# intel/QATzip

Hardware: AMD Instinct MI355X
Metric: compress + decompress GB/s (input bytes), QZ_DEFLATE_GZIP_EXT L1, 64 KB chunks (higher is better)
Workload: dtype u8

## Files before the change

### qatzip_amd/csrc/qzd_inflate.hip

```cpp
#include <algorithm>
#include <atomic>
#include <chrono>
#include <condition_variable>
#include <functional>
#include <mutex>
#include <thread>
#include <string.h>
#include <string>
#include <vector>

#include "qzd_internal.h"
#include <stdlib.h>
#include "qzk_inflate.h"
#include "qzk_inflate_lane.h"
#include "qzk_inflate_spec.h"
#include "qzk_checksum.h"
#include "qzd_inflate_plan.h"
#include <stddef.h>

static_assert(sizeof(qzp_seg) == sizeof(qzk_infseg) && offsetof(qzp_seg, in_off) == offsetof(qzk_infseg, in_off) &&
              offsetof(qzp_seg, out_off) == offsetof(qzk_infseg, out_off) && offsetof(qzp_seg, in_len) == offsetof(qzk_infseg, in_len) &&
              offsetof(qzp_seg, out_cap) == offsetof(qzk_infseg, out_cap) && offsetof(qzp_seg, flags) == offsetof(qzk_infseg, flags) &&
              offsetof(qzp_seg, pad) == offsetof(qzk_infseg, pad), "qzp_seg mirrors qzk_infseg");
static_assert(sizeof(qzp_res) == sizeof(qzk_infres) && offsetof(qzp_res, status) == offsetof(qzk_infres, status) &&
              offsetof(qzp_res, in_used) == offsetof(qzk_infres, in_used) && offsetof(qzp_res, out_len) == offsetof(qzk_infres, out_len) &&
              offsetof(qzp_res, nblocks) == offsetof(qzk_infres, nblocks), "qzp_res mirrors qzk_infres");
static_assert(QZP_FINAL == QZK_INF_FINAL && QZP_FLUSH == QZK_INF_FLUSH && QZP_TOKSEG_BYTES == sizeof(qzk_tokseg), "qzd_inflate_plan.h's constants");

#define QZD_LANE_MIN_SEGS 1024u
#define QZD_LANE_MIN_SEGS_BIG 2048u
#define QZD_LANE_MIN(seg_bytes) ((seg_bytes) <= 65536u + 64u ? QZD_LANE_MIN_SEGS : QZD_LANE_MIN_SEGS_BIG)
#define QZD_LANE_SEGS_PER_WAVE 16u
#define QZD_SPEC_LANES 4u
#define QZD_SPEC_LANES_FEW 8u
#define QZD_SPEC_FEW_SEGS 16384u
#define QZD_SPEC_FEW_SEGS_BIG 32768u
#define QZD_SPEC_LANES_FEWER 16u
#define QZD_SPEC_FEWER_SEGS 8192u
static uint32_t spec_lanes(const qzk_infseg *hs, uint32_t nsegs)
{
    const bool big = hs[0].out_cap > 16384u + 64u, upto512 = hs[0].out_cap <= 524288u + 64u;
    uint32_t K = nsegs <= QZD_SPEC_FEWER_SEGS && hs[0].out_cap > 131072u + 64u && upto512 ? 32u
// ... 98 lines not shown
struct tp_host { qzk_infseg *segs; qzk_infres *res; qzk_tokseg *ts; uint32_t *ord; };
static tp_host tp_host_of(qzd_ctx *c, const tp_mirror &M)
{
    return tp_host{(qzk_infseg *)c->h_aux, (qzk_infres *)(c->h_aux + M.o_res), (qzk_tokseg *)(c->h_aux + M.o_ts), (uint32_t *)(c->h_aux + M.o_ord)};
}
struct tp_dev {
    qzk_infseg *segs; qzk_infres *res; qzk_inf_tab *tab; qzk_tokseg *ts; qzk_chain *ch; qzk_rec *rec;
    uint8_t *lit; qzk_seq *seq; uint32_t *ord;
};

struct tp_plan {
    bool uniform; qzk_tsfill F;
    uint64_t arena;
    uint64_t hb0, hb_rg; uint32_t R;
};
static int plan_regions(qzd_ctx *c, const qzk_infseg *hs, uint32_t nsegs, uint32_t K, qzk_tokseg *tsv, tp_plan *pl)
{
    uint64_t arena = 0, max_cap = 0;
    qzk_tsfill &F = pl->F;
    bool uniform = nsegs > 0 && K <= 32;
    for (uint32_t i = 0; i < nsegs && uniform; i++) uniform = !(hs[i].flags & QZK_INF_COUNT_ONLY) && hs[i].out_cap == hs[0].out_cap;
    if (uniform) {
        F.seg = 0; max_cap = hs[0].out_cap;
        for (uint32_t j = 0; j < K; j++) {
            F.len[j] = K == 1 ? QZK_TOK_REGION(hs[0].out_cap) : QZK_SPEC_REGION(hs[0].out_cap, K, j);
            F.pre[j] = F.seg; F.seg += F.len[j];
        }
        arena = (uint64_t)nsegs * F.seg;
    } else
    for (uint32_t i = 0; i < nsegs; i++) {
        const bool writes = !(hs[i].flags & QZK_INF_COUNT_ONLY);
        if (writes && hs[i].out_cap > max_cap) max_cap = hs[i].out_cap;
        for (uint32_t j = 0; j < K; j++) {
            const uint64_t rg = !writes ? 0 : K == 1 ? QZK_TOK_REGION(hs[i].out_cap) : QZK_SPEC_REGION(hs[i].out_cap, K, j);
            tsv[(size_t)i * K + j].lit_off = arena; tsv[(size_t)i * K + j].seq_off = (arena + rg) / 8;
            arena += rg;
        }
    }
    pl->uniform = uniform;
    pl->R = K == 1 ? 0u : std::min<uint32_t>(nsegs, QZK_SPEC_HANDBACK(nsegs));
    pl->hb0 = arena; pl->hb_rg = QZK_TOK_REGION(max_cap);
    pl->arena = arena + (uint64_t)pl->R * pl->hb_rg;
    bool aligned = ((pl->hb0 | pl->hb_rg) & 15) == 0;
    if (uniform) for (uint32_t j = 0; j < K; j++) aligned &= ((F.pre[j] | F.len[j] | F.seg) & 15) == 0;
    else for (size_t i = 0; i < (size_t)nsegs * K; i++) aligned &= ((tsv[i].lit_off & 15) | (tsv[i].seq_off & 1)) == 0;
    if (!aligned) { snprintf(c->err, sizeof(c->err), "inflate: a token region is not 16-byte aligned"); return QZD_ERR_PARAM; }
    return QZD_OK;
}
static void fill_host(const tp_plan &pl, qzk_tokseg *tsv, uint32_t nsegs, uint32_t K)
{
    for (uint32_t i = 0; i < nsegs; i++)
        for (uint32_t j = 0; j < K; j++) {
            const uint64_t a = (uint64_t)i * pl.F.seg + pl.F.pre[j];
            tsv[(size_t)i * K + j].lit_off = a; tsv[(size_t)i * K + j].seq_off = (a + pl.F.len[j]) / 8;
        }
// ... 9 lines not shown
    c->d_big = NULL; c->big_cap = 0;
    const char *cap_e = getenv("QATZIP_AMD_SCRATCH_MAX");
    const bool refused = cap_e && need > (size_t)strtoull(cap_e, NULL, 10);
    if (refused || hipMalloc(&c->d_big, need) != hipSuccess) {
        (void)hipGetLastError();
        c->d_big = NULL;
        return QZD_ERR_NOMEM;
    }
    c->big_cap = need;
    return QZD_OK;
}

#ifndef QZD_TOK_OCC
#define QZD_TOK_OCC 2
#endif
static void tok_launch(hipStream_t st, const uint8_t *d_comp, const tp_dev &D, uint32_t nsegs, uint32_t K, const uint32_t *order, uint32_t count)
{
    uint32_t lpw = QZD_LANE_SEGS_PER_WAVE;
    const char *le = getenv("QATZIP_AMD_INFLATE_LPW");
    if (le) { int v = atoi(le); if (v == 8 || v == 16 || v == 32 || v == 64) lpw = (uint32_t)v; }
    const char *oe = getenv("QATZIP_AMD_INFLATE_OCC");
    const int occ = oe ? atoi(oe) : 0;
    const dim3 grid(((order ? count : nsegs) + lpw - 1) / lpw), blk(lpw);
#define QZD_TOK_LAUNCH(N, W) hipLaunchKernelGGL((qzk_inflate_tok_kernel<N, W>), grid, blk, 0, st, d_comp, D.segs, D.res, nsegs, D.tab, \
                                               D.ts, D.lit, D.seq, D.ch, order, count, K)
    switch (lpw) {
    case 8: if (occ == 2) QZD_TOK_LAUNCH(8, 2); else QZD_TOK_LAUNCH(8, 4); break;
    case 32: QZD_TOK_LAUNCH(32, 1); break;
    case 64: QZD_TOK_LAUNCH(64, 1); break;
    default: QZD_TOK_LAUNCH(16, QZD_TOK_OCC);
    }
#undef QZD_TOK_LAUNCH
}
static void spec_launch(qzd_ctx *c, hipStream_t st, const uint8_t *d_comp, const tp_dev &D, const qzk_infseg *hs, uint32_t nsegs, uint32_t K)
{
    const uint32_t spw = 64 / K;
    const dim3 grid((nsegs + spw - 1) / spw), blk(64);
    static std::atomic<uint64_t> spec_epoch{0};
    const uint64_t epoch = ++spec_epoch;
    uint32_t over = hs[0].out_cap > 65536u + 64u ? 2u : nsegs <= 4096u ? 1u : 1000u;
// ... 67 lines not shown
        c->so_sent = off[parts];
    }
    return QZD_OK;
}

static int fetch_results(qzd_ctx *c, qzk_infres *st_res, const qzk_infres *d_res, uint32_t nsegs, qzk_infres *h_res, hipStream_t st)
{
    const size_t rb = (size_t)nsegs * sizeof(qzk_infres);
    HIPCHK(c, ctl_copy(st_res, d_res, rb, st));
    HIPCHK(c, hipStreamSynchronize(st));
    HIPCHK(c, hipGetLastError());
    memcpy(h_res, st_res, rb);
    return QZD_OK;
}

static int two_phase(qzd_ctx *c, const uint8_t *d_comp, uint8_t *d_out, const qzk_infseg *hs, uint32_t nsegs,
                     qzk_infres *h_res, uint32_t K, hipStream_t st, bool run_b = true)
{
    const tp_mirror M = tp_mirror_of(nsegs, K);
    int rc = qzd_aux_reserve(c, M.bytes + 64);
    if (rc) return rc;
    const tp_host H = tp_host_of(c, M);
    const size_t sb = (size_t)nsegs * sizeof(qzk_infseg);
    memcpy(H.segs, hs, sb);
    tp_plan pl;
    rc = plan_regions(c, hs, nsegs, K, H.ts, &pl);
    if (rc) return rc;
    const size_t tabb = ((size_t)nsegs * sizeof(qzk_inf_tab) + 255) & ~(size_t)255;
    const size_t tsb = ((size_t)nsegs * K * sizeof(qzk_tokseg) + 255) & ~(size_t)255;
    const size_t chb = ((size_t)nsegs * sizeof(qzk_chain) + 255) & ~(size_t)255;
    const size_t rcb = K == 1 ? 0 : (((size_t)nsegs * K * QZK_SPEC_NREC * sizeof(qzk_rec) + 255) & ~(size_t)255);
    const size_t litb = (pl.arena + 1023) & ~(uint64_t)255;
    const size_t ordb = ((size_t)nsegs * 4 + 255) & ~(size_t)255;
    const size_t need = tabb + tsb + chb + rcb + litb + ordb + 256;
    const bool stream_out = run_b && c->so_host && c->so_nat && nsegs >= QZD_LANE_MIN_SEGS;
    if (big_reserve(c, need, st) != QZD_OK) {
        if (K > 1) return two_phase(c, d_comp, d_out, hs, nsegs, h_res, 1, st, run_b);
        snprintf(c->err, sizeof(c->err), "inflate: %zu bytes of decode scratch are not available", need);
        return QZD_ERR_NOMEM;
    }
    tp_dev D;
    uint8_t *pb = c->d_big;
    D.segs = (qzk_infseg *)c->d_aux; D.res = (qzk_infres *)(c->d_aux + M.o_res);
    D.tab = (qzk_inf_tab *)pb; pb += tabb;
    D.ts = (qzk_tokseg *)pb; pb += tsb;
    D.ch = (qzk_chain *)pb; pb += chb;
    D.rec = (qzk_rec *)pb; pb += rcb;
    D.lit = pb; pb += litb;
    D.seq = (qzk_seq *)D.lit;
    D.ord = (uint32_t *)pb;
    HIPCHK(c, ctl_copy(D.segs, H.segs, sb, st));
    if (pl.uniform) {
        hipLaunchKernelGGL(qzk_ts_fill_kernel, dim3((unsigned)std::min<size_t>(((size_t)nsegs * K + 255) / 256, 1024)), dim3(256), 0, st, D.ts, nsegs, K, pl.F);
        HIPCHK(c, hipGetLastError());
    } else HIPCHK(c, ctl_copy(D.ts, H.ts, (size_t)nsegs * K * sizeof(qzk_tokseg), st));
    HIPCHK(c, hipEventRecord(c->ev[1][1], st));
    bool res_fresh = false;
    if (K == 1) tok_launch(st, d_comp, D, nsegs, K, NULL, 0);
    else {
        spec_launch(c, st, d_comp, D, hs, nsegs, K);
        uint32_t nredo = 0;
        rc = handback_redo(c, st, d_comp, pl, H, D, nsegs, K, &nredo);
        if (rc) return rc;
        if (nredo > pl.R) {
            c->inf_k1rerun_acc++;
            return two_phase(c, d_comp, d_out, hs, nsegs, h_res, 1, st, run_b);
        }
        res_fresh = nredo == 0;
    }
    HIPCHK(c, hipEventRecord(c->ev[1][0], st));
// ... 260 lines not shown
}

static void build_candidates(const std::vector<uint32_t> &start, uint64_t n, uint32_t avail, uint32_t shift, uint32_t seg_hint,
                             std::vector<qzk_infseg> &ps, std::vector<uint32_t> &where)
{
    const uint32_t ns = (uint32_t)ps.size();
    std::vector<uint32_t> order(ns);
    order_by_clen(start, n, shift, order);
    for (uint32_t i = 0; i < ns; i++) {
        const uint32_t k = order[i];
        where[k] = i;
        ps[i].in_off = start[k]; ps[i].in_len = avail - start[k];
        ps[i].out_off = 0; ps[i].out_cap = seg_hint; ps[i].flags = 0; ps[i].pad = clen(start.data(), (uint32_t)start.size(), n, k);
    }
}
static void seat_links(const qzp_walk &W, const std::vector<uint32_t> &where, std::vector<qzk_infseg> &ps, std::vector<uint32_t> &chain)
{
    for (qzk_infseg &s : ps) s.flags = QZK_INF_COUNT_ONLY;
    for (const qzp_link &l : W.links) {
        qzk_infseg &s = ps[where[l.cand]];
        s.out_off = l.out_off; s.out_cap = l.out_len; s.flags = 0;
        chain.push_back(where[l.cand]);
    }
}

#define QZD_PATH_DONE 1
#define QZD_PATH_NEXT 2
#define QZD_PATH_LANES_NOMEM 3
struct inf_lap {
    bool on; std::chrono::steady_clock::time_point prev;
    void operator()(const char *what)
    {
        if (!on) return;
        auto t = std::chrono::steady_clock::now();
        fprintf(stderr, "[qzd_inflate_stream] %-22s %8.3f ms\n", what, std::chrono::duration<double, std::milli>(t - prev).count());
        prev = t;
    }
};
struct inf_call {
    qzd_ctx *c; const uint8_t *d_src; uint64_t n; uint8_t *d_dst; uint64_t dst_cap; uint32_t seg_hint;
    uint8_t *h_dst; int *h_sent;
    bool scan_ok; std::vector<uint32_t> start; uint32_t ns;
    bool lanes, lanes_nomem;
    std::vector<qzk_infseg> segs; std::vector<qzk_infres> res;
    uint64_t total_out, total_in;
    inf_lap lap;
};

static int path_lanes(inf_call &S)
{
    qzd_ctx *c = S.c;
    const uint32_t ns = S.ns;
    static const bool lone_lanes = getenv("QATZIP_AMD_LONE_WAVE") == NULL;
    if (!(S.scan_ok && S.seg_hint && (ns > 1 || (lone_lanes && S.seg_hint > 16384u)) && S.lanes)) return QZD_PATH_NEXT;
    static const uint32_t cls_shift = cls_shift_of(getenv("QATZIP_AMD_INFLATE_CLS"));
    std::vector<qzk_infseg> ps(ns);
    std::vector<qzk_infres> pr(ns);
    std::vector<uint32_t> where(ns);
    build_candidates(S.start, S.n, (uint32_t)S.n, cls_shift, S.seg_hint, ps, where);
    S.lap("segment records");
    HIPCHK(c, hipEventRecord(c->ev[0][0], c->st[0]));
    int rc = two_phase(c, S.d_src, S.d_dst, ps.data(), ns, pr.data(), spec_lanes(ps.data(), ns), c->st[0], false);
    if (rc == QZD_ERR_NOMEM) return QZD_PATH_LANES_NOMEM;
    if (rc) return rc;
    S.lap("phase A");
    const qzp_walk W = chain_walk(S.start.data(), ns, ns, (const qzp_res *)pr.data(), where.data(), 0, 0, S.dst_cap);
    if (!W.ok) return QZD_PATH_NEXT;
    if (W.over < W.links.size()) return QZD_ERR_DSTCAP;
    std::vector<uint32_t> chain;
    seat_links(W, where, ps, chain);
    c->so_sent = 0;
    rc = two_phase_resolve(c, S.d_src, S.d_dst, ps.data(), ns, chain.data(), (uint32_t)chain.size(), pr.data(), S.h_dst, c->st[0]);
    if (rc) return rc;
    bool ok = true;
    for (uint32_t i : chain) if (pr[i].status < 0) { ok = false; break; }
    HIPCHK(c, hipEventRecord(c->ev[0][1], c->st[0]));
    HIPCHK(c, hipStreamSynchronize(c->st[0]));
    float t = 0;
    if (hipEventElapsedTime(&t, c->ev[0][0], c->ev[0][1]) == hipSuccess) c->inf_ms[0] += t;
    S.lap("phase B");
// ... 83 lines not shown
}

static int inflate_stream(qzd_ctx *c, const uint8_t *d_src, uint64_t n, uint8_t *d_dst, uint64_t dst_cap,
                          uint32_t seg_hint, uint64_t *h_in_used, uint64_t *h_out_len, uint32_t *h_crc, uint8_t *h_dst, int *h_sent)
{
    if (h_sent) *h_sent = 0;
    if (!c || !d_src || !h_in_used || !h_out_len) return QZD_ERR_PARAM;
    if (n == 0 || n > 0xffffffffull) return QZD_ERR_PARAM;
    hipSetDevice(c->device);
    c->inf_ms[0] = c->inf_ms[1] = c->inf_ms[2] = c->inf_ms[3] = 0;
    *h_in_used = 0; *h_out_len = 0;
    static const bool trace = getenv("QATZIP_AMD_TRACE") != NULL;
    inf_call S;
    S.c = c; S.d_src = d_src; S.n = n; S.d_dst = d_dst; S.dst_cap = dst_cap; S.seg_hint = seg_hint; S.h_dst = h_dst; S.h_sent = h_sent;
    S.total_out = S.total_in = 0;
    S.lap.on = trace; S.lap.prev = std::chrono::steady_clock::now();
    std::vector<uint32_t> mk;
    int rc = find_markers(c, d_src, n, mk);
    S.lap("marker scan + sort");
    if (rc < 0) return rc;
    S.scan_ok = rc == 0;
    S.start.push_back(0);
    if (S.scan_ok) for (uint32_t p : mk) if (p < n) S.start.push_back(p);
    S.ns = (uint32_t)S.start.size();
    const char *force_path = getenv("QATZIP_AMD_INFLATE");
    S.lanes = force_path ? force_path[0] == 'l' : true;
    S.lanes_nomem = false;
    rc = path_lanes(S);
    if (rc == QZD_PATH_LANES_NOMEM) { S.lanes_nomem = true; rc = QZD_PATH_NEXT; }
    if (rc == QZD_PATH_NEXT) { S.segs.resize(S.ns); S.res.resize(S.ns); rc = path_optimistic(S); }
    if (rc == QZD_PATH_NEXT) rc = path_two_pass(S);
    if (rc == QZD_PATH_NEXT) rc = path_one_wave(S);
    if (rc != QZD_PATH_DONE) return rc;
    *h_in_used = S.total_in; *h_out_len = S.total_out;
    S.lap("chain check / rest");
    if (h_crc) { rc = qzd_crc32(c, d_dst, S.total_out, h_crc); S.lap("crc32"); return rc; }
    return QZD_OK;
}

extern "C" int qzd_inflate_stream(qzd_ctx *c, const uint8_t *d_src, uint64_t n, uint8_t *d_dst, uint64_t dst_cap,
                                  uint32_t seg_hint, uint64_t *h_in_used, uint64_t *h_out_len, uint32_t *h_crc)
{
    return inflate_stream(c, d_src, n, d_dst, dst_cap, seg_hint, h_in_used, h_out_len, h_crc, NULL, NULL);
}

extern "C" int qzd_inflate_stream_to_host(qzd_ctx *c, const uint8_t *d_src, uint64_t n, uint8_t *d_dst, uint64_t dst_cap,
                                          uint32_t seg_hint, uint64_t *h_in_used, uint64_t *h_out_len, uint32_t *h_crc,
                                          uint8_t *h_dst, int *h_sent)
{
    if (!h_dst || !h_sent) return QZD_ERR_PARAM;
// ... 256 lines not shown
```

### qatzip_amd/csrc/qzd_inflate_plan.h

```cpp
#ifndef QZD_INFLATE_PLAN_H
#define QZD_INFLATE_PLAN_H
#include <stdint.h>
#include <stdlib.h>
#include <algorithm>
#include <vector>

struct qzp_seg { uint64_t in_off, out_off; uint32_t in_len, out_cap, flags, pad; };
struct qzp_res { int32_t status; uint32_t in_used, out_len, nblocks; };
#define QZP_FINAL 0
#define QZP_FLUSH 1
#define QZP_TOKSEG_BYTES 16u

static inline uint32_t clen(const uint32_t *start, uint32_t ns, uint64_t n, uint32_t k)
{
    return (k + 1 < ns ? start[k + 1] : (uint32_t)n) - start[k];
}

#define QZP_CLASSES 8192u
static inline void order_by_clen(const std::vector<uint32_t> &start, uint64_t n, uint32_t shift, std::vector<uint32_t> &order)
{
    const uint32_t ns = (uint32_t)order.size(), nstart = (uint32_t)start.size();
    std::vector<uint32_t> cnt(QZP_CLASSES + 1, 0);
    auto rcls = [&](uint32_t k) { const uint32_t v = clen(start.data(), nstart, n, k) >> shift; return QZP_CLASSES - 1 - (v < QZP_CLASSES ? v : QZP_CLASSES - 1); };
    for (uint32_t i = 0; i < ns; i++) cnt[rcls(i) + 1]++;
    for (uint32_t i = 0; i < QZP_CLASSES; i++) cnt[i + 1] += cnt[i];
    for (uint32_t i = 0; i < ns; i++) order[cnt[rcls(i)]++] = i;
// ... 27 lines not shown
        W.links.push_back(qzp_link{k, oo, r.out_len});
        oo += r.out_len;
        if (oo > cap && W.over == (size_t)-1) W.over = W.links.size() - 1;
        if (r.status == QZP_FINAL) { W.final = true; W.total_in = (uint64_t)start[k] + r.in_used; break; }
        W.next = start[k] + r.in_used;
        uint32_t j = k + 1;
        while (j < nstart && start[j] < W.next) j++;
        if (j >= nstart || start[j] != W.next) { W.ok = false; break; }
        k = j;
    }
    W.oo = oo;
    if (W.over == (size_t)-1) W.over = W.links.size();
    return W;
}

#define QZD_PIPE_MAX 8u
#define QZD_PIPE_FIRST_PCT 3u
#define QZD_PIPE_MIN_BYTES (12u << 20)
#define QZD_PIPE_GROW_NUM 9u
#define QZD_PIPE_GROW_DEN 5u
static inline void pipe_plan(uint64_t n, uint64_t cut[QZD_PIPE_MAX + 1], uint32_t *P_out)
{
    uint64_t len = std::max<uint64_t>(n * QZD_PIPE_FIRST_PCT / 100, QZD_PIPE_MIN_BYTES), at = 0;
    uint32_t P = 0;
    cut[0] = 0;
    while (P + 1 < QZD_PIPE_MAX && at + len + len / 2 < n) {
        at = (at + len) & ~(uint64_t)4095; cut[++P] = at;
        len = len * QZD_PIPE_GROW_NUM / QZD_PIPE_GROW_DEN;
    }
    cut[++P] = n;
// ... 36 lines not shown
```

### qatzip_amd/csrc/qzk_checksum.h

```cpp
#ifndef QZK_CHECKSUM_H
#define QZK_CHECKSUM_H
#include "qzk_deflate_huff.h"

typedef struct { uint64_t off; uint32_t len; uint32_t pad; } qzk_range;

QZ_KERNEL qzk_crc_kernel(const uint8_t *data, const qzk_range *ranges, uint32_t nranges, uint32_t *crc_out)
{
    QZ_LDS qzk_crc_lds S;
    const uint32_t r = blockIdx.x;
    if (r >= nranges) return;
    const uint32_t c = qzk_block_crc32(&S, data + ranges[r].off, ranges[r].len);
    if (threadIdx.x == 0) crc_out[r] = c;
}

QZ_KERNEL qzk_crc_chunks_kernel(const uint8_t *src, uint64_t src_len, uint32_t chunk_sz, uint32_t nchunks, uint32_t *crc_out,
                                const uint32_t *cdesc )
{
    QZ_LDS qzk_crc_lds S;
    const uint32_t c = blockIdx.x;
    if (c >= nchunks) return;
    const uint64_t off = (uint64_t)c * chunk_sz;
    const uint32_t n = cdesc ? (cdesc[c] & 0x7fffffffu) : (uint32_t)((src_len - off) < chunk_sz ? (src_len - off) : chunk_sz);
    const uint32_t v = qzk_block_crc32(&S, src + off, n);
    if (threadIdx.x == 0) crc_out[c] = v;
}

#define QZK_ADLER_MOD 65521u
QZ_KERNEL qzk_adler_chunks_kernel(const uint8_t *src, uint64_t src_len, uint32_t chunk_sz, uint32_t nchunks, uint32_t *out)
{
    QZ_LDS uint32_t pa[QZK_HT], pb[QZK_HT];
    const uint32_t c = blockIdx.x, t = threadIdx.x;
    if (c >= nchunks) return;
    const uint64_t off = (uint64_t)c * chunk_sz;
    const uint32_t n = (uint32_t)((src_len - off) < chunk_sz ? (src_len - off) : chunk_sz);
    const uint32_t S = (n + QZK_HT - 1) / QZK_HT;
    const uint32_t b0 = t * S < n ? t * S : n, b1 = (t + 1) * S < n ? (t + 1) * S : n;
// ... 18 lines not shown
```

### qatzip_amd/csrc/qzk_inflate_lane.h

```cpp
#ifndef QZK_INFLATE_LANE_H
#define QZK_INFLATE_LANE_H
#include "qzk_inflate.h"
#include "qzk_lz_batch.h"

#ifdef QZ_SIM
#define QZK_PIN(x) ((void)0)
#else
#define QZK_PIN(x) asm volatile("" : "+v"(x))
#endif

#ifndef QZK_LLROOT
#define QZK_LLROOT 9
#endif
#ifndef QZK_LDROOT
#define QZK_LDROOT 7
#endif
#define QZK_CLROOT 7
#define QZK_SIDE_BYTES 256
#define QZK_SIDE_SPARE 28
#define QZK_LPOOL_N (QZK_SIDE_BYTES - (1 << QZK_LDROOT) - QZK_SIDE_SPARE)
#define QZK_LANE_ROOTSZ ((1 << QZK_LLROOT) + QZK_SIDE_BYTES / 2)
#define QZK_DROOT8(droot) ((uint8_t *)(droot))
#define QZK_LPOOL(droot) ((uint8_t *)(droot) + (1 << QZK_LDROOT))

// ... 85 lines not shown
    for (int l = rootbits + 1; l <= maxlen; l++) {
        code = (code << 1) | (uint32_t)(bits & 1); bits >>= 1;
        if (l > b->bc) return -1;
        const uint32_t c = count[l], f = first[l];
        if (c && code >= f && code - f < c) { QZK_DROP(b, l); return sorted[index[l] + code - f]; }
    }
    return -1;
}

typedef struct __attribute__((packed, aligned(1))) { uint64_t v; } qz_u64u;
QZ_DEV uint64_t qzk_ld64u(const uint8_t *p) { return ((const qz_u64u *)p)->v; }
QZ_DEV void qzk_st64u(uint8_t *p, uint64_t v) { ((qz_u64u *)p)->v = v; }

typedef struct { uint32_t litrun; uint16_t mlen; uint16_t dm1; } qzk_seq;
typedef struct { uint64_t lit_off; uint64_t seq_off; } qzk_tokseg;
#define QZK_SPEC_MAXK 8
#define QZK_INF_ESPEC (-6)
#define QZK_PIECE_RAW 0xffffffffu
typedef struct { uint32_t sub, seq_first, seq_count, lit_first, lrun_skip; } qzk_chain_el;
#ifndef QZK_CHAIN_MAXEL
#define QZK_CHAIN_MAXEL 640
#endif
typedef struct { uint32_t nel, pad; qzk_chain_el el[QZK_CHAIN_MAXEL]; } qzk_chain;
#define QZK_TOK_LITCAP(out_cap) ((((uint64_t)(out_cap) + 31) & ~(uint64_t)31) + 32)
#define QZK_TOK_SEQCAP(out_cap) (((uint64_t)(out_cap) / 3 + 3) & ~(uint64_t)1)
#define QZK_TOK_REGION(out_cap) (QZK_TOK_LITCAP(out_cap) + 8 * QZK_TOK_SEQCAP(out_cap))
static_assert(QZK_TOK_REGION(1) % 16 == 0 && QZK_TOK_REGION(1000) % 16 == 0 && QZK_TOK_REGION(16384 + 64) % 16 == 0 &&
              QZK_TOK_REGION(65536) % 16 == 0 && QZK_TOK_REGION(65536 + 64) % 16 == 0 && QZK_TOK_REGION(131072 + 64) % 16 == 0 &&
              QZK_TOK_REGION(524288 + 64) % 16 == 0 && QZK_TOK_REGION(0xffffffffu) % 16 == 0, "a sub-stream region must end 16-aligned");

// ... 568 lines not shown
        lv |= run ? (e2 >> 4) << (8 * lk) : 0u;
        lk += run ? 1u : 0u;
    }
    static_assert(NX <= 3, "a trip's literals are one dword of the staging");
    (void)lv_hi;
    if (nrec) qzk_tok_seq_rec(O, rec);
    qzk_tok_lits4(O, lv, lk);
    S->op += lk;
    S->b.bb = bb; S->b.bc = bc;
}

template <int LPW, int OCC = 2>
QZ_KERNEL_OCC(64, OCC) qzk_inflate_tok_kernel(const uint8_t *comp, const qzk_infseg *segs, qzk_infres *res, uint32_t nsegs,
                                 qzk_inf_tab *tabs, const qzk_tokseg *ts, uint8_t *lits, qzk_seq *seqs,
                                 qzk_chain *chains, const uint32_t *order = 0 ,
                                 uint32_t count = 0, uint32_t ts_stride = 1 )
{
    QZ_LDS uint16_t roots[LPW][QZK_LANE_ROOTSZ];
    const uint32_t widx = blockIdx.x * LPW + threadIdx.x;
    if (widx >= (order ? count : nsegs)) return;
    const uint32_t sidx = order ? order[widx] : widx;
    if (sidx >= nsegs) return;
    const qzk_infseg sg = segs[sidx];
    qzk_inf_tab *T = tabs + sidx;
    uint16_t *const lroot = roots[threadIdx.x], *const droot = lroot + (1 << QZK_LLROOT);
    qzk_lane_st S;
    S.b.p = comp + sg.in_off; S.b.end = sg.in_len; qzk_lseek(&S.b, 0);
    S.op = 0; S.nblocks = 0; S.last = 0; S.clen = 0; S.rpos = 0; S.out_cap = sg.out_cap;
    S.lmax = 0; S.dmax = 0; S.lbase = 0; S.status = QZK_INF_EDATA; S.state = QZK_LS_HDR;
    S.through = sg.flags & QZK_INF_THROUGH_FLUSH;
    qzk_tok_out O;
    {
        const bool co = sg.flags & QZK_INF_COUNT_ONLY;
// ... 89 lines not shown

#define QZK_RSYNC() qz_wave_sync()

#ifdef QZK_SPEC_PROF
__device__ unsigned long long qzk_stamp_b[2];
#endif
#ifndef QZK_RES_WAVES
#define QZK_RES_WAVES 1
#endif
#ifndef QZK_RES_OCC
#define QZK_RES_OCC 8
#endif

QZ_KERNEL_OCC(64 * QZK_RES_WAVES, QZK_RES_OCC) qzk_lz_resolve_kernel(const uint8_t *comp, uint8_t *out, const qzk_infseg *segs, qzk_infres *res, uint32_t nsegs,
                                const qzk_tokseg *ts, uint32_t ts_stride, const uint8_t *lits, const qzk_seq *seqs,
                                const qzk_chain *chains, const uint32_t *order , uint32_t count)
{
    QZ_LDS __attribute__((aligned(16))) uint8_t obuf_all[QZK_RES_WAVES][QZK_RB_OB];
    QZ_LDS __attribute__((aligned(16))) uint8_t lbuf_all[QZK_RES_WAVES][QZK_RB_LT];
#ifdef QZK_SPEC_PROF
    if ((threadIdx.x & 63) == 0) atomicMin(&qzk_stamp_b[0], (unsigned long long)__builtin_amdgcn_s_memrealtime());
#endif
    const int lane = qz_lane();
    const uint32_t widx = blockIdx.x * QZK_RES_WAVES + (threadIdx.x >> 6);
    if (widx >= (order ? count : nsegs)) return;
    const uint32_t sidx = qz_uniform(order ? order[widx] : widx);
    if (sidx >= nsegs) return;
    const qzk_infseg sg = segs[sidx];
    if (res[sidx].status < 0 || (sg.flags & QZK_INF_COUNT_ONLY)) return;
    qzk_rb S;
    qzk_rb_init(&S, obuf_all[threadIdx.x >> 6], lbuf_all[threadIdx.x >> 6], out + sg.out_off,
                (sg.flags & QZK_INF_THROUGH_FLUSH) ? sg.out_off : 0 , sg.out_cap);
    const uint32_t nel = chains[sidx].nel;
    int err = 0;
    for (uint32_t e = 0; e < nel && !err; e++) {
        const qzk_chain_el ce = chains[sidx].el[e];
        if (ce.sub == QZK_PIECE_RAW) {
            if ((uint64_t)S.obase + ce.seq_count > sg.out_cap) { err = QZK_INF_EOUT; break; }
            qzk_rb_flush(&S, lane);
// ... 27 lines not shown
                lbase += L; b0 += 1;
                cur = b0 + (uint32_t)lane < ns ? qzk_rb_ld64((const uint8_t *)(sq - b0 - lane)) : 0;
                continue;
            }
            const uint64_t nxt = b0 + n + (uint32_t)lane < ns ? qzk_rb_ld64((const uint8_t *)(sq - b0 - n - lane)) : 0;
            if ((uint32_t)lane >= n) { s_tot -= litrun + mlen; s_lit -= litrun; litrun = 0; mlen = 0; }
            const uint32_t Tb = qz_readlane(s_tot, (int)n - 1), Lb = qz_readlane(s_lit, (int)n - 1);
            err = qzk_rb_batch(&S, lp + lbase, Lb, s_lit - litrun, litrun, mlen, dist, s_tot, Tb, lane);
            if (err) break;
            lbase += Lb; b0 += n;
            cur = nxt;
        }
    }
    if (!err) qzk_rb_flush(&S, lane);
    if (err) res[sidx].status = err;
}

#endif
```

Before: 66.30.

## Move inflate chain walk, link seating and CRC onto device in one pass

Adds a device-side path that runs speculative phase A, builds the handback list, gathers candidates, walks the segment chain, seats links, resolves LZ output and computes chunked CRC entirely on the GPU stream. It replaces the host round-trips for results, the host chain walk and seat_links, plus the separate CRC pass, with a single synchronize. The costs are several small serial kernels, including a single-workgroup chain walk. When the device walk cannot finish, the code falls back to the host path after fetching results.

```diff
diff --git a/qatzip_amd/csrc/qzd_inflate.hip b/qatzip_amd/csrc/qzd_inflate.hip
--- a/qatzip_amd/csrc/qzd_inflate.hip
+++ b/qatzip_amd/csrc/qzd_inflate.hip
@@ -14,6 +14,7 @@
 #include "qzk_inflate.h"
 #include "qzk_inflate_lane.h"
 #include "qzk_inflate_spec.h"
+#include "qzk_inflate_plan.h"
 #include "qzk_checksum.h"
 #include "qzd_inflate_plan.h"
 #include <stddef.h>
@@ -25,7 +26,8 @@
 static_assert(sizeof(qzp_res) == sizeof(qzk_infres) && offsetof(qzp_res, status) == offsetof(qzk_infres, status) &&
               offsetof(qzp_res, in_used) == offsetof(qzk_infres, in_used) && offsetof(qzp_res, out_len) == offsetof(qzk_infres, out_len) &&
               offsetof(qzp_res, nblocks) == offsetof(qzk_infres, nblocks), "qzp_res mirrors qzk_infres");
-static_assert(QZP_FINAL == QZK_INF_FINAL && QZP_FLUSH == QZK_INF_FLUSH && QZP_TOKSEG_BYTES == sizeof(qzk_tokseg), "qzd_inflate_plan.h's constants");
+static_assert(QZP_FINAL == QZK_INF_FINAL && QZP_FLUSH == QZK_INF_FLUSH && QZP_TOKSEG_BYTES == sizeof(qzk_tokseg) && QZP_COUNT_ONLY == QZK_INF_COUNT_ONLY,
+              "qzd_inflate_plan.h's constants");
 
 #define QZD_LANE_MIN_SEGS 1024u
 #define QZD_LANE_MIN_SEGS_BIG 2048u
@@ -154,6 +156,7 @@
     uint64_t arena;
     uint64_t hb0, hb_rg; uint32_t R;
 };
+static uint32_t handback_regions(uint32_t nsegs, uint32_t K) { return K == 1 ? 0u : std::min<uint32_t>(nsegs, QZK_SPEC_HANDBACK(nsegs)); }
 static int plan_regions(qzd_ctx *c, const qzk_infseg *hs, uint32_t nsegs, uint32_t K, qzk_tokseg *tsv, tp_plan *pl)
 {
     uint64_t arena = 0, max_cap = 0;
@@ -178,7 +181,7 @@
         }
     }
     pl->uniform = uniform;
-    pl->R = K == 1 ? 0u : std::min<uint32_t>(nsegs, QZK_SPEC_HANDBACK(nsegs));
+    pl->R = handback_regions(nsegs, K);
     pl->hb0 = arena; pl->hb_rg = QZK_TOK_REGION(max_cap);
     pl->arena = arena + (uint64_t)pl->R * pl->hb_rg;
     bool aligned = ((pl->hb0 | pl->hb_rg) & 15) == 0;
@@ -218,7 +221,8 @@
 #ifndef QZD_TOK_OCC
 #define QZD_TOK_OCC 2
 #endif
-static void tok_launch(hipStream_t st, const uint8_t *d_comp, const tp_dev &D, uint32_t nsegs, uint32_t K, const uint32_t *order, uint32_t count)
+static void tok_launch(hipStream_t st, const uint8_t *d_comp, const tp_dev &D, uint32_t nsegs, uint32_t K, const uint32_t *order, uint32_t count,
+                       const qzk_inf_plan *plan = NULL )
 {
     uint32_t lpw = QZD_LANE_SEGS_PER_WAVE;
     const char *le = getenv("QATZIP_AMD_INFLATE_LPW");
@@ -227,7 +231,7 @@
     const int occ = oe ? atoi(oe) : 0;
     const dim3 grid(((order ? count : nsegs) + lpw - 1) / lpw), blk(lpw);
 #define QZD_TOK_LAUNCH(N, W) hipLaunchKernelGGL((qzk_inflate_tok_kernel<N, W>), grid, blk, 0, st, d_comp, D.segs, D.res, nsegs, D.tab, \
-                                               D.ts, D.lit, D.seq, D.ch, order, count, K)
+                                               D.ts, D.lit, D.seq, D.ch, order, count, K, plan)
     switch (lpw) {
     case 8: if (occ == 2) QZD_TOK_LAUNCH(8, 2); else QZD_TOK_LAUNCH(8, 4); break;
     case 32: QZD_TOK_LAUNCH(32, 1); break;
@@ -325,11 +329,100 @@
     return QZD_OK;
 }
 
+struct tp_devwalk {
+    const uint32_t *start, *where;
+    uint64_t dst_cap; uint32_t seg_hint; bool want_crc;
+    qzk_inf_plan plan;
+    bool have_crc; uint32_t crc;
+};
+#define QZD_CRC_PIECE (256u * 1024u)
+struct dw_layout { size_t o_plan, o_crc, o_hb, o_start, o_where, o_cand, o_loff, bytes; uint32_t nr; uint64_t out_max; };
+static dw_layout dw_layout_of(const tp_mirror &M, uint32_t nsegs, uint32_t R, const tp_devwalk &dw)
+{
+    auto up16 = [](size_t v) { return (v + 15) & ~(size_t)15; };
+    dw_layout L;
+    L.out_max = std::min<uint64_t>(dw.dst_cap, (uint64_t)nsegs * dw.seg_hint);
+    L.nr = dw.want_crc ? (uint32_t)((L.out_max + QZD_CRC_PIECE - 1) / QZD_CRC_PIECE) : 0u;
+    L.o_plan = (M.bytes + 255) & ~(size_t)255;
+    L.o_crc = L.o_plan + sizeof(qzk_inf_plan);
+    L.o_hb = L.o_crc + up16((size_t)L.nr * 4);
+    L.o_start = L.o_hb + up16((size_t)R * 4);
+    L.o_where = L.o_start + up16((size_t)nsegs * 4);
+    L.o_cand = L.o_where + up16((size_t)nsegs * 4);
+    L.o_loff = L.o_cand + (size_t)nsegs * sizeof(qzk_cand);
+    L.bytes = L.o_loff + (size_t)nsegs * 8;
+    return L;
+}
+
 static int two_phase(qzd_ctx *c, const uint8_t *d_comp, uint8_t *d_out, const qzk_infseg *hs, uint32_t nsegs,
-                     qzk_infres *h_res, uint32_t K, hipStream_t st, bool run_b = true)
+                     qzk_infres *h_res, uint32_t K, hipStream_t st, bool run_b, tp_devwalk *dw);
+static int devwalk_run(qzd_ctx *c, hipStream_t st, const uint8_t *d_comp, uint8_t *d_out, const qzk_infseg *hs, uint32_t nsegs, qzk_infres *h_res,
+                       uint32_t K, const tp_mirror &M, const tp_dev &D, const tp_plan &pl, tp_devwalk *dw)
+{
+    const dw_layout L = dw_layout_of(M, nsegs, pl.R, *dw);
+    uint8_t *const dp = c->d_aux, *const hp = c->h_aux;
+    qzk_inf_plan *const d_plan = (qzk_inf_plan *)(dp + L.o_plan);
+    uint32_t *const d_hb = (uint32_t *)(dp + L.o_hb), *const d_start = (uint32_t *)(dp + L.o_start), *const d_where = (uint32_t *)(dp + L.o_where);
+    qzk_cand *const d_cand = (qzk_cand *)(dp + L.o_cand);
+    uint64_t *const d_loff = (uint64_t *)(dp + L.o_loff);
+    memcpy(hp + L.o_start, dw->start, (size_t)nsegs * 4);
+    memcpy(hp + L.o_where, dw->where, (size_t)nsegs * 4);
+    HIPCHK(c, ctl_copy(d_start, hp + L.o_start, L.o_cand - L.o_start, st));
+    HIPCHK(c, hipEventRecord(c->ev[1][1], st));
+    if (K == 1) tok_launch(st, d_comp, D, nsegs, K, NULL, 0);
+    else spec_launch(c, st, d_comp, D, hs, nsegs, K);
+    hipLaunchKernelGGL(qzk_handback_list_kernel, dim3(1), dim3(QZK_PLAN_WG), 0, st, (const qzk_infres *)D.res, K == 1 ? 0u : nsegs, pl.R, K,
+                       pl.hb0, pl.hb_rg, D.ts, d_hb, d_plan);
+    if (K > 1) tok_launch(st, d_comp, D, nsegs, K, d_hb, pl.R, d_plan);
+    HIPCHK(c, hipEventRecord(c->ev[1][0], st));
+    hipLaunchKernelGGL(qzk_cand_gather_kernel, dim3((nsegs + 255) / 256), dim3(256), 0, st, (const qzk_infres *)D.res, (const uint32_t *)d_where, nsegs,
+                       d_cand, d_loff, D.segs, (const qzk_inf_plan *)d_plan);
+    hipLaunchKernelGGL(qzk_chain_walk_kernel, dim3(1), dim3(QZK_PLAN_WG), 0, st, (const uint32_t *)d_start, nsegs, (const qzk_cand *)d_cand, dw->dst_cap,
+                       d_loff, D.ord, d_plan);
+    hipLaunchKernelGGL(qzk_seat_links_kernel, dim3((nsegs + 255) / 256), dim3(256), 0, st, (const qzk_cand *)d_cand, (const uint64_t *)d_loff, nsegs,
+                       D.segs, (const qzk_inf_plan *)d_plan);
+    HIPCHK(c, hipEventRecord(c->ev[1][3], st));
+    hipLaunchKernelGGL(qzk_lz_resolve_kernel, dim3((nsegs + QZK_RES_WAVES - 1) / QZK_RES_WAVES), dim3(64 * QZK_RES_WAVES), 0, st,
+                       d_comp, d_out, (const qzk_infseg *)D.segs, D.res, nsegs, (const qzk_tokseg *)D.ts, K, (const uint8_t *)D.lit, (const qzk_seq *)D.seq,
+                       (const qzk_chain *)D.ch, (const uint32_t *)D.ord, 0u, d_plan);
+    HIPCHK(c, hipEventRecord(c->ev[1][2], st));
+    HIPCHK(c, hipEventRecord(c->ev[0][1], st));
+    if (L.nr) {
+        HIPCHK(c, hipEventRecord(c->ev[0][2], st));
+        hipLaunchKernelGGL(qzk_crc_chunks_kernel, dim3(L.nr), dim3(QZK_HT), 0, st, (const uint8_t *)d_out, L.out_max, QZD_CRC_PIECE, L.nr,
+                           (uint32_t *)(dp + L.o_crc), (const uint32_t *)NULL, (const uint64_t *)&d_plan->crc_len);
+        HIPCHK(c, hipEventRecord(c->ev[0][3], st));
+    }
+    HIPCHK(c, ctl_copy(hp + L.o_plan, d_plan, L.o_hb - L.o_plan, st));
+    HIPCHK(c, hipStreamSynchronize(st));
+    HIPCHK(c, hipGetLastError());
+    c->tp.segs = D.segs; c->tp.res = D.res; c->tp.ts = D.ts; c->tp.lits = D.lit; c->tp.seqs = D.seq; c->tp.chains = D.ch;
+    c->tp.ord = D.ord; c->tp.nsegs = nsegs; c->tp.K = K;
+    dw->plan = *(const qzk_inf_plan *)(hp + L.o_plan);
+    c->inf_handback_acc += dw->plan.nredo;
+    float t = 0;
+    if (hipEventElapsedTime(&t, c->ev[1][1], c->ev[1][0]) == hipSuccess) c->inf_ms[3] += t;
+    if (dw->plan.hb_over) {
+        c->inf_k1rerun_acc++;
+        return two_phase(c, d_comp, d_out, hs, nsegs, h_res, 1, st, false, dw);
+    }
+    if (!dw->plan.go) return QZD_OK;
+    if (hipEventElapsedTime(&t, c->ev[1][3], c->ev[1][2]) == hipSuccess) c->inf_ms[2] += t;
+    if (hipEventElapsedTime(&t, c->ev[0][0], c->ev[0][1]) == hipSuccess) c->inf_ms[0] += t;
+    const uint32_t nr = (uint32_t)((dw->plan.oo + QZD_CRC_PIECE - 1) / QZD_CRC_PIECE);
+    if (L.nr && nr <= L.nr && !dw->plan.b_err) {
+        dw->crc = qzd_crc32_fold((const uint32_t *)(hp + L.o_crc), nr, QZD_CRC_PIECE, dw->plan.oo);
+        dw->have_crc = true;
+        if (hipEventElapsedTime(&t, c->ev[0][2], c->ev[0][3]) == hipSuccess) c->inf_ms[1] += t;
+    }
+    return QZD_OK;
+}
+
+static int two_phase(qzd_ctx *c, const uint8_t *d_comp, uint8_t *d_out, const qzk_infseg *hs, uint32_t nsegs,
+                     qzk_infres *h_res, uint32_t K, hipStream_t st, bool run_b = true, tp_devwalk *dw = NULL )
 {
     const tp_mirror M = tp_mirror_of(nsegs, K);
-    int rc = qzd_aux_reserve(c, M.bytes + 64);
+    int rc = qzd_aux_reserve(c, (dw ? dw_layout_of(M, nsegs, handback_regions(nsegs, K), *dw).bytes : M.bytes) + 64);
     if (rc) return rc;
     const tp_host H = tp_host_of(c, M);
     const size_t sb = (size_t)nsegs * sizeof(qzk_infseg);
@@ -346,7 +439,7 @@
     const size_t need = tabb + tsb + chb + rcb + litb + ordb + 256;
     const bool stream_out = run_b && c->so_host && c->so_nat && nsegs >= QZD_LANE_MIN_SEGS;
     if (big_reserve(c, need, st) != QZD_OK) {
-        if (K > 1) return two_phase(c, d_comp, d_out, hs, nsegs, h_res, 1, st, run_b);
+        if (K > 1) return two_phase(c, d_comp, d_out, hs, nsegs, h_res, 1, st, run_b, dw);
         snprintf(c->err, sizeof(c->err), "inflate: %zu bytes of decode scratch are not available", need);
         return QZD_ERR_NOMEM;
     }
@@ -365,6 +458,7 @@
         hipLaunchKernelGGL(qzk_ts_fill_kernel, dim3((unsigned)std::min<size_t>(((size_t)nsegs * K + 255) / 256, 1024)), dim3(256), 0, st, D.ts, nsegs, K, pl.F);
         HIPCHK(c, hipGetLastError());
     } else HIPCHK(c, ctl_copy(D.ts, H.ts, (size_t)nsegs * K * sizeof(qzk_tokseg), st));
+    if (dw) return devwalk_run(c, st, d_comp, d_out, hs, nsegs, h_res, K, M, D, pl, dw);
     HIPCHK(c, hipEventRecord(c->ev[1][1], st));
     bool res_fresh = false;
     if (K == 1) tok_launch(st, d_comp, D, nsegs, K, NULL, 0);
@@ -655,15 +749,6 @@
         ps[i].out_off = 0; ps[i].out_cap = seg_hint; ps[i].flags = 0; ps[i].pad = clen(start.data(), (uint32_t)start.size(), n, k);
     }
 }
-static void seat_links(const qzp_walk &W, const std::vector<uint32_t> &where, std::vector<qzk_infseg> &ps, std::vector<uint32_t> &chain)
-{
-    for (qzk_infseg &s : ps) s.flags = QZK_INF_COUNT_ONLY;
-    for (const qzp_link &l : W.links) {
-        qzk_infseg &s = ps[where[l.cand]];
-        s.out_off = l.out_off; s.out_cap = l.out_len; s.flags = 0;
-        chain.push_back(where[l.cand]);
-    }
-}
 
 #define QZD_PATH_DONE 1
 #define QZD_PATH_NEXT 2
@@ -685,6 +770,7 @@
     bool lanes, lanes_nomem;
     std::vector<qzk_infseg> segs; std::vector<qzk_infres> res;
     uint64_t total_out, total_in;
+    bool want_crc, have_crc; uint32_t crc;
     inf_lap lap;
 };
 
@@ -696,15 +782,39 @@
     if (!(S.scan_ok && S.seg_hint && (ns > 1 || (lone_lanes && S.seg_hint > 16384u)) && S.lanes)) return QZD_PATH_NEXT;
     static const uint32_t cls_shift = cls_shift_of(getenv("QATZIP_AMD_INFLATE_CLS"));
     std::vector<qzk_infseg> ps(ns);
-    std::vector<qzk_infres> pr(ns);
+    std::vector<qzk_infres> pr;
     std::vector<uint32_t> where(ns);
     build_candidates(S.start, S.n, (uint32_t)S.n, cls_shift, S.seg_hint, ps, where);
     S.lap("segment records");
     HIPCHK(c, hipEventRecord(c->ev[0][0], c->st[0]));
-    int rc = two_phase(c, S.d_src, S.d_dst, ps.data(), ns, pr.data(), spec_lanes(ps.data(), ns), c->st[0], false);
-    if (rc == QZD_ERR_NOMEM) return QZD_PATH_LANES_NOMEM;
-    if (rc) return rc;
-    S.lap("phase A");
+    const uint32_t K = spec_lanes(ps.data(), ns);
+    const char *hw = getenv("QATZIP_AMD_INFLATE_HOSTWALK");
+    int rc;
+    if (!S.h_dst && !(hw && hw[0] && hw[0] != '0')) {
+        tp_devwalk dw;
+        dw.start = S.start.data(); dw.where = where.data(); dw.dst_cap = S.dst_cap; dw.seg_hint = S.seg_hint; dw.want_crc = S.want_crc;
+        dw.have_crc = false; dw.crc = 0;
+        rc = two_phase(c, S.d_src, S.d_dst, ps.data(), ns, pr.data(), K, c->st[0], false, &dw);
+        if (rc == QZD_ERR_NOMEM) return QZD_PATH_LANES_NOMEM;
+        if (rc) return rc;
+        S.lap("A + walk + B + crc");
+        if (S.lap.on) fprintf(stderr, "[qzd_inflate_stream] %u candidates, %u links, %u handed back\n", ns, dw.plan.nlinks, dw.plan.nredo);
+        if (dw.plan.go) {
+            if (dw.plan.b_err) return QZD_PATH_NEXT;
+            S.total_out = dw.plan.oo; S.total_in = dw.plan.total_in;
+            S.have_crc = dw.have_crc; S.crc = dw.crc;
+            return QZD_PATH_DONE;
+        }
+        pr.resize(ns);
+        rc = fetch_results(c, tp_host_of(c, tp_mirror_of(ns, c->tp.K)).res, (const qzk_infres *)c->tp.res, ns, pr.data(), c->st[0]);
+        if (rc) return rc;
+    } else {
+        pr.resize(ns);
+        rc = two_phase(c, S.d_src, S.d_dst, ps.data(), ns, pr.data(), K, c->st[0], false);
+        if (rc == QZD_ERR_NOMEM) return QZD_PATH_LANES_NOMEM;
+        if (rc) return rc;
+        S.lap("phase A");
+    }
     const qzp_walk W = chain_walk(S.start.data(), ns, ns, (const qzp_res *)pr.data(), where.data(), 0, 0, S.dst_cap);
     if (!W.ok) return QZD_PATH_NEXT;
     if (W.over < W.links.size()) return QZD_ERR_DSTCAP;
@@ -818,6 +928,7 @@
     inf_call S;
     S.c = c; S.d_src = d_src; S.n = n; S.d_dst = d_dst; S.dst_cap = dst_cap; S.seg_hint = seg_hint; S.h_dst = h_dst; S.h_sent = h_sent;
     S.total_out = S.total_in = 0;
+    S.want_crc = h_crc != NULL; S.have_crc = false; S.crc = 0;
     S.lap.on = trace; S.lap.prev = std::chrono::steady_clock::now();
     std::vector<uint32_t> mk;
     int rc = find_markers(c, d_src, n, mk);
@@ -838,6 +949,7 @@
     if (rc != QZD_PATH_DONE) return rc;
     *h_in_used = S.total_in; *h_out_len = S.total_out;
     S.lap("chain check / rest");
+    if (h_crc && S.have_crc) { *h_crc = S.crc; return QZD_OK; }
     if (h_crc) { rc = qzd_crc32(c, d_dst, S.total_out, h_crc); S.lap("crc32"); return rc; }
     return QZD_OK;
 }
diff --git a/qatzip_amd/csrc/qzd_inflate_plan.h b/qatzip_amd/csrc/qzd_inflate_plan.h
--- a/qatzip_amd/csrc/qzd_inflate_plan.h
+++ b/qatzip_amd/csrc/qzd_inflate_plan.h
@@ -10,6 +10,7 @@
 #define QZP_FINAL 0
 #define QZP_FLUSH 1
 #define QZP_TOKSEG_BYTES 16u
+#define QZP_COUNT_ONLY 1u
 
 static inline uint32_t clen(const uint32_t *start, uint32_t ns, uint64_t n, uint32_t k)
 {
@@ -67,6 +68,17 @@
     return W;
 }
 
+template <class SEG>
+static inline void seat_links(const qzp_walk &W, const std::vector<uint32_t> &where, std::vector<SEG> &ps, std::vector<uint32_t> &chain)
+{
+    for (SEG &s : ps) s.flags = QZP_COUNT_ONLY;
+    for (const qzp_link &l : W.links) {
+        SEG &s = ps[where[l.cand]];
+        s.out_off = l.out_off; s.out_cap = l.out_len; s.flags = 0;
+        chain.push_back(where[l.cand]);
+    }
+}
+
 #define QZD_PIPE_MAX 8u
 #define QZD_PIPE_FIRST_PCT 3u
 #define QZD_PIPE_MIN_BYTES (12u << 20)
diff --git a/qatzip_amd/csrc/qzk_checksum.h b/qatzip_amd/csrc/qzk_checksum.h
--- a/qatzip_amd/csrc/qzk_checksum.h
+++ b/qatzip_amd/csrc/qzk_checksum.h
@@ -14,12 +14,17 @@
 }
 
 QZ_KERNEL qzk_crc_chunks_kernel(const uint8_t *src, uint64_t src_len, uint32_t chunk_sz, uint32_t nchunks, uint32_t *crc_out,
-                                const uint32_t *cdesc )
+                                const uint32_t *cdesc ,
+                                const uint64_t *dev_len = 0 )
 {
     QZ_LDS qzk_crc_lds S;
     const uint32_t c = blockIdx.x;
     if (c >= nchunks) return;
     const uint64_t off = (uint64_t)c * chunk_sz;
+    if (dev_len) {
+        if (*dev_len < src_len) src_len = *dev_len;
+        if (off >= src_len) return;
+    }
     const uint32_t n = cdesc ? (cdesc[c] & 0x7fffffffu) : (uint32_t)((src_len - off) < chunk_sz ? (src_len - off) : chunk_sz);
     const uint32_t v = qzk_block_crc32(&S, src + off, n);
     if (threadIdx.x == 0) crc_out[c] = v;
diff --git a/qatzip_amd/csrc/qzk_inflate_lane.h b/qatzip_amd/csrc/qzk_inflate_lane.h
--- a/qatzip_amd/csrc/qzk_inflate_lane.h
+++ b/qatzip_amd/csrc/qzk_inflate_lane.h
@@ -123,6 +123,13 @@
 
 typedef struct { uint32_t litrun; uint16_t mlen; uint16_t dm1; } qzk_seq;
 typedef struct { uint64_t lit_off; uint64_t seq_off; } qzk_tokseg;
+
+typedef struct {
+    uint32_t nredo, hb_over, ok, final;
+    uint64_t total_in, oo;
+    uint32_t nlinks, over, go, b_err;
+    uint64_t crc_len, pad;
+} qzk_inf_plan;
 #define QZK_SPEC_MAXK 8
 #define QZK_INF_ESPEC (-6)
 #define QZK_PIECE_RAW 0xffffffffu
@@ -721,9 +728,14 @@
 QZ_KERNEL_OCC(64, OCC) qzk_inflate_tok_kernel(const uint8_t *comp, const qzk_infseg *segs, qzk_infres *res, uint32_t nsegs,
                                  qzk_inf_tab *tabs, const qzk_tokseg *ts, uint8_t *lits, qzk_seq *seqs,
                                  qzk_chain *chains, const uint32_t *order = 0 ,
-                                 uint32_t count = 0, uint32_t ts_stride = 1 )
+                                 uint32_t count = 0, uint32_t ts_stride = 1 ,
+                                 const qzk_inf_plan *plan = 0 )
 {
     QZ_LDS uint16_t roots[LPW][QZK_LANE_ROOTSZ];
+    if (plan) {
+        if (plan->hb_over) return;
+        count = plan->nredo;
+    }
     const uint32_t widx = blockIdx.x * LPW + threadIdx.x;
     if (widx >= (order ? count : nsegs)) return;
     const uint32_t sidx = order ? order[widx] : widx;
@@ -843,7 +855,8 @@
 
 QZ_KERNEL_OCC(64 * QZK_RES_WAVES, QZK_RES_OCC) qzk_lz_resolve_kernel(const uint8_t *comp, uint8_t *out, const qzk_infseg *segs, qzk_infres *res, uint32_t nsegs,
                                 const qzk_tokseg *ts, uint32_t ts_stride, const uint8_t *lits, const qzk_seq *seqs,
-                                const qzk_chain *chains, const uint32_t *order , uint32_t count)
+                                const qzk_chain *chains, const uint32_t *order , uint32_t count,
+                                qzk_inf_plan *plan = 0 )
 {
     QZ_LDS __attribute__((aligned(16))) uint8_t obuf_all[QZK_RES_WAVES][QZK_RB_OB];
     QZ_LDS __attribute__((aligned(16))) uint8_t lbuf_all[QZK_RES_WAVES][QZK_RB_LT];
@@ -852,6 +865,10 @@
 #endif
     const int lane = qz_lane();
     const uint32_t widx = blockIdx.x * QZK_RES_WAVES + (threadIdx.x >> 6);
+    if (plan) {
+        if (!plan->go) return;
+        count = plan->nlinks;
+    }
     if (widx >= (order ? count : nsegs)) return;
     const uint32_t sidx = qz_uniform(order ? order[widx] : widx);
     if (sidx >= nsegs) return;
@@ -909,6 +926,7 @@
     }
     if (!err) qzk_rb_flush(&S, lane);
     if (err) res[sidx].status = err;
-}
-
-#endif
+    if (err && plan) plan->b_err = 1;
+}
+
+#endif
diff --git a/qatzip_amd/csrc/qzk_inflate_plan.h b/qatzip_amd/csrc/qzk_inflate_plan.h
--- /dev/null
+++ b/qatzip_amd/csrc/qzk_inflate_plan.h
@@ -0,0 +1,201 @@
+#ifndef QZK_INFLATE_PLAN_H
+#define QZK_INFLATE_PLAN_H
+#include "qzk_inflate_lane.h"
+
+#define QZK_PLAN_WG 1024u
+
+typedef struct { int32_t status; uint32_t in_used; uint32_t out_len; uint32_t where; } qzk_cand;
+
+QZ_DEV void qzk_plan_wsum(const uint32_t *w, int wv, uint32_t *before, uint32_t *total)
+{
+    uint32_t b = 0, s = 0;
+    for (int i = 0; i < (int)(QZK_PLAN_WG / 64); i++) { if (i < wv) b += w[i]; s += w[i]; }
+    *before = b; *total = s;
+}
+
+QZ_KERNEL_MAX(QZK_PLAN_WG) qzk_handback_list_kernel(const qzk_infres *res, uint32_t nscan, uint32_t R, uint32_t K, uint64_t hb0,
+                                                    uint64_t hb_rg, qzk_tokseg *ts, uint32_t *list, qzk_inf_plan *P)
+{
+    QZ_LDS uint32_t wc[2][QZK_PLAN_WG / 64];
+    const uint32_t t = threadIdx.x;
+    const int lane = (int)(t & 63), wv = (int)(t >> 6);
+    uint32_t mine = 0;
+    for (uint32_t i = t; i < nscan; i += QZK_PLAN_WG) mine += res[i].status == QZK_INF_ESPEC;
+    const uint32_t im = qz_wave_incl_scan(mine);
+    if (lane == 63) wc[0][wv] = im;
+    qz_block_sync();
+    uint32_t before, total;
+    qzk_plan_wsum(wc[0], wv, &before, &total);
+    if (t == 0) {
+        qzk_inf_plan p;
+        p.nredo = total; p.hb_over = total > R; p.ok = 0; p.final = 0; p.total_in = 0; p.oo = 0; p.nlinks = 0; p.over = 0;
+        p.go = 0; p.b_err = 0; p.crc_len = 0; p.pad = 0;
+        *P = p;
+    }
+    if (total == 0 || total > R) return;
+    uint32_t done = 0;
+    for (uint32_t base = 0, it = 1; base < nscan; base += QZK_PLAN_WG, it++) {
+        const uint32_t i = base + t;
+        const bool hb = i < nscan && res[i].status == QZK_INF_ESPEC;
+        const uint64_t m = qz_ballot(hb);
+        if (lane == 0) wc[it & 1][wv] = (uint32_t)qz_popc64(m);
+        qz_block_sync();
+        qzk_plan_wsum(wc[it & 1], wv, &before, &total);
+        if (hb) {
+            const uint32_t k = done + before + (uint32_t)qz_popc64(m & qz_below(lane));
+            list[k] = i;
+            qzk_tokseg t0;
+            t0.lit_off = hb0 + (uint64_t)k * hb_rg; t0.seq_off = (hb0 + (uint64_t)(k + 1) * hb_rg) / 8;
+            ts[(uint64_t)i * K] = t0;
+        }
+        done += total;
+    }
+}
+
+#define QZK_NO_LINK (~0ull)
+QZ_KERNEL_MAX(256) qzk_cand_gather_kernel(const qzk_infres *res, const uint32_t *where, uint32_t ns, qzk_cand *cand, uint64_t *loff,
+                                          qzk_infseg *segs, const qzk_inf_plan *P)
+{
+    if (P->hb_over) return;
+    for (uint32_t k = blockIdx.x * blockDim.x + threadIdx.x; k < ns; k += gridDim.x * blockDim.x) {
+        const uint32_t w = where[k];
+        const qzk_infres r = res[w];
+        qzk_cand c; c.status = r.status; c.in_used = r.in_used; c.out_len = r.out_len; c.where = w;
+        cand[k] = c;
+        loff[k] = QZK_NO_LINK;
+        segs[w].flags = QZK_INF_COUNT_ONLY;
+    }
+}
+QZ_KERNEL_MAX(256) qzk_seat_links_kernel(const qzk_cand *cand, const uint64_t *loff, uint32_t ns, qzk_infseg *segs, const qzk_inf_plan *P)
+{
+    if (P->hb_over) return;
+    for (uint32_t k = blockIdx.x * blockDim.x + threadIdx.x; k < ns; k += gridDim.x * blockDim.x) {
+        const uint64_t o = loff[k];
+        if (o == QZK_NO_LINK) continue;
+        qzk_infseg *s = segs + cand[k].where;
+        s->out_off = o; s->out_cap = cand[k].out_len; s->flags = 0;
+    }
+}
+
+#define QZK_WALK_NONE 0xffffffffu
+typedef struct { uint64_t oo, total_in; uint32_t cur, nlinks, over, done; } qzk_walk_st;
+QZ_KERNEL_MAX(QZK_PLAN_WG) qzk_chain_walk_kernel(const uint32_t *start, uint32_t ns, const qzk_cand *cand, uint64_t dst_cap,
+                                                 uint64_t *loff, uint32_t *ord, qzk_inf_plan *P)
+{
+    QZ_LDS uint32_t wlo[2][QZK_PLAN_WG / 64], whi[2][QZK_PLAN_WG / 64], wbad[2][QZK_PLAN_WG / 64];
+    QZ_LDS uint32_t s_start[QZK_PLAN_WG + 1], s_used[QZK_PLAN_WG], s_len[QZK_PLAN_WG], s_where[QZK_PLAN_WG];
+    QZ_LDS int32_t s_stat[QZK_PLAN_WG];
+    QZ_LDS uint64_t s_pre[QZK_PLAN_WG + 1], s_badm[QZK_PLAN_WG / 64], s_roo[QZK_PLAN_WG];
+    QZ_LDS uint32_t s_rf[QZK_PLAN_WG], s_rcnt[QZK_PLAN_WG], s_rnl[QZK_PLAN_WG], s_nruns;
+    QZ_LDS qzk_walk_st s_w;
+    if (P->hb_over) return;
+    const uint32_t t = threadIdx.x;
+    const int lane = (int)(t & 63), wv = (int)(t >> 6);
+    qzk_walk_st W;
+    W.oo = 0; W.total_in = 0; W.cur = 0; W.nlinks = 0; W.over = QZK_WALK_NONE; W.done = 0;
+    qzk_cand cn; cn.status = QZK_INF_EDATA; cn.in_used = 0; cn.out_len = 0; cn.where = 0;
+    uint32_t sn0 = 0, sn1 = 0;
+    if (t < ns) { cn = cand[t]; sn0 = start[t]; sn1 = t + 1 < ns ? start[t + 1] : 0; }
+    for (uint32_t base = 0, it = 0; base < ns && !W.done; base += QZK_PLAN_WG, it++) {
+        const uint32_t k = base + t, tile_end = ns - base < QZK_PLAN_WG ? ns : base + QZK_PLAN_WG;
+        const bool live = k < ns;
+        const qzk_cand cd = cn;
+        const uint32_t st0 = sn0, st1 = sn1;
+        if (k + QZK_PLAN_WG < ns) {
+            const uint32_t kn = k + QZK_PLAN_WG;
+            cn = cand[kn]; sn0 = start[kn]; sn1 = kn + 1 < ns ? start[kn + 1] : 0;
+        }
+        if (W.cur >= tile_end) continue;
+        const bool regular = !live || (k + 1 < ns ? cd.status == QZK_INF_FLUSH && st0 + cd.in_used == st1 : cd.status == QZK_INF_FINAL);
+        const uint32_t lo = live ? cd.out_len & 0xffffu : 0u, hi = live ? cd.out_len >> 16 : 0u;
+        const uint32_t ilo = qz_wave_incl_scan(lo), ihi = qz_wave_incl_scan(hi);
+        const uint64_t bad = qz_ballot(!regular);
+        if (lane == 63) { wlo[it & 1][wv] = ilo; whi[it & 1][wv] = ihi; }
+        if (lane == 0) wbad[it & 1][wv] = bad != 0;
+        qz_block_sync();
+        uint32_t blo, tlo, bhi, thi, bb, anybad;
+        qzk_plan_wsum(wlo[it & 1], wv, &blo, &tlo);
+        qzk_plan_wsum(whi[it & 1], wv, &bhi, &thi);
+        qzk_plan_wsum(wbad[it & 1], wv, &bb, &anybad);
+        const uint64_t tile_out = (uint64_t)tlo + ((uint64_t)thi << 16);
+        if (W.cur == base && !anybad && !(W.over == QZK_WALK_NONE && W.oo + tile_out > dst_cap)) {
+            if (live) {
+                loff[k] = W.oo + (uint64_t)(blo + ilo - lo) + ((uint64_t)(bhi + ihi - hi) << 16);
+                ord[W.nlinks + t] = cd.where;
+            }
+            W.oo += tile_out; W.nlinks += tile_end - base; W.cur = tile_end;
+            if (tile_end == ns) {
+                if (k == ns - 1) { s_w.total_in = (uint64_t)st0 + cd.in_used; }
+                qz_block_sync();
+                W.done = 1; W.total_in = s_w.total_in;
+            }
+            continue;
+        }
+        const uint64_t pre = (uint64_t)(blo + ilo - lo) + ((uint64_t)(bhi + ihi - hi) << 16);
+        s_pre[t] = pre;
+        if (t == QZK_PLAN_WG - 1) s_pre[QZK_PLAN_WG] = tile_out;
+        if (lane == 0) s_badm[wv] = bad;
+        if (live) { s_start[t] = st0; s_used[t] = cd.in_used; s_len[t] = cd.out_len; s_where[t] = cd.where; s_stat[t] = cd.status; }
+        if (live && k + 1 == tile_end && k + 1 < ns) s_start[t + 1] = st1;
+        qz_block_sync();
+        if (t == 0) {
+            uint32_t c = W.cur, nruns = 0;
+            const uint32_t tlen = tile_end - base;
+            while (c < tile_end) {
+                const uint32_t i = c - base;
+                uint32_t w = i >> 6;
+                uint64_t m = s_badm[w] & ~qz_below((int)(i & 63));
+                while (!m && ++w < QZK_PLAN_WG / 64) m = s_badm[w];
+                uint32_t b = m ? w * 64 + (uint32_t)qz_ctz64(m) : tlen;
+                if (b > tlen) b = tlen;
+                if (b > i) {
+                    const uint64_t run_out = s_pre[b] - s_pre[i];
+                    if (W.over == QZK_WALK_NONE && W.oo + run_out > dst_cap) {
+                        uint32_t x0 = i, x1 = b - 1;
+                        while (x0 < x1) { const uint32_t xm = (x0 + x1) / 2; if (W.oo + (s_pre[xm + 1] - s_pre[i]) > dst_cap) x1 = xm; else x0 = xm + 1; }
+                        W.over = W.nlinks + (x0 - i);
+                    }
+                    s_rf[nruns] = i; s_rcnt[nruns] = b - i; s_roo[nruns] = W.oo; s_rnl[nruns] = W.nlinks; nruns++;
+                    W.oo += run_out; W.nlinks += b - i; c = base + b;
+                    if (c == ns) { W.done = 1; W.total_in = (uint64_t)s_start[b - 1] + s_used[b - 1]; break; }
+                    continue;
+                }
+                if (s_stat[i] != QZK_INF_FINAL && s_stat[i] != QZK_INF_FLUSH) { W.done = 2; break; }
+                loff[c] = W.oo;
+                ord[W.nlinks] = s_where[i];
+                W.oo += s_len[i];
+                if (W.oo > dst_cap && W.over == QZK_WALK_NONE) W.over = W.nlinks;
+                W.nlinks++;
+                if (s_stat[i] == QZK_INF_FINAL) { W.done = 1; W.total_in = (uint64_t)s_start[i] + s_used[i]; break; }
+                const uint32_t next = s_start[i] + s_used[i];
+                uint32_t j = c + 1, sj = 0;
+                while (j < ns && j <= base + QZK_PLAN_WG && (sj = s_start[j - base]) < next) j++;
+                if (j < ns && j > base + QZK_PLAN_WG) {
+                    uint32_t a = j, b = ns;
+                    while (a < b) { const uint32_t m = a + (b - a) / 2; if (start[m] < next) a = m + 1; else b = m; }
+                    j = a;
+                    if (j < ns) sj = start[j];
+                }
+                if (j >= ns || sj != next) { W.done = 2; break; }
+                c = j;
+            }
+            W.cur = c;
+            s_w = W; s_nruns = nruns;
+        }
+        qz_block_sync();
+        W = s_w;
+        for (uint32_t r = 0, nr = s_nruns; r < nr; r++) {
+            const uint32_t f = s_rf[r];
+            if (t >= f && t < f + s_rcnt[r]) { loff[k] = s_roo[r] + (pre - s_pre[f]); ord[s_rnl[r] + (t - f)] = cd.where; }
+        }
+        qz_block_sync();
+    }
+    if (t == 0) {
+        const uint32_t ok = W.done == 1, over = W.over == QZK_WALK_NONE ? W.nlinks : W.over;
+        P->ok = ok; P->final = ok; P->total_in = W.total_in; P->oo = W.oo; P->nlinks = W.nlinks; P->over = over;
+        P->go = ok && over == W.nlinks;
+        P->crc_len = ok && over == W.nlinks ? W.oo : 0;
+    }
+}
+
+#endif
```

Result: no change. 66.88 (median of 6 runs) (+0.9%).
